# gregspangenberg/shoulder

Measured on AMD Instinct MI355X. Metric: humerus meshes/s end-to-end (all 4 landmarks), higher is better.
Workload: dtype f64 geometry + bf16 UNet

## Files before the change

shoulder_amd/csrc/k_ovf.h:

```cpp
#pragma once
#include "k_slices.h"

namespace sh {

struct OvfPools {
  Seg* segs; double* ring; unsigned char* work;
  unsigned long long seg_cap, ring_cap, work_cap;
  unsigned long long* ctr;
  int open_mode;
};
__host__ __device__ inline int ovf_nodes(int cnt, int open_mode) { return open_mode ? 2 * cnt : cnt; }

struct OvfSet { long long* soff; long long* roff; long long* woff; int* fill; int* list; int* nlist ; int* list2; };

__host__ __device__ inline unsigned ovf_hash_size(int n) { unsigned h = 64; while (h < 2u * (unsigned)n) h <<= 1; return h; }
__host__ __device__ inline unsigned long long ovf_work_bytes(int n) {
  unsigned long long b = (unsigned long long)n * 8ull * 5ull + (unsigned long long)ovf_hash_size(n) * 4ull + (unsigned long long)n * 4ull * 6ull + 64ull;
  const unsigned long long te = (unsigned long long)(n + 1) * 8ull * 7ull + 64ull;
  if (te > b) b = te;
  return (b + 15ull) & ~15ull;
}

__global__ void k_ovf_plan(int N, int nplanes, const int* __restrict__ seg_count, OvfPools P, OvfSet S, int* __restrict__ err) {
  const int pl = blockIdx.x * blockDim.x + threadIdx.x;
// ... 277 lines not shown
      const int qq = q == L ? 0 : q;
      const int src = rev ? (qq == 0 ? 0 : L - qq) : qq;
      ring_out[2 * q] = rx[o + src];
      ring_out[2 * q + 1] = ry[o + src];
    }
  }
  __syncthreads();
}

template <bool OPEN>
__global__ void __launch_bounds__(SH_HUGE_THREADS)
k_slice_link_huge(int N, const int* __restrict__ seg_count, OvfPools P, OvfSet S, double* __restrict__ centroids, double* __restrict__ areas,
                  int* __restrict__ nloops, int* __restrict__ ring_n, int want_ring, int select, int* __restrict__ err, double* __restrict__ areas_total,
                  const double* __restrict__ vobb, const long long* __restrict__ voff, const double* __restrict__ zeff, const OpenCfg oc) {
  const int nl = *S.nlist;
  for (int i = blockIdx.x; i < nl; i += gridDim.x) {
    const int pl = S.list[i];
    slice_link_plane_g<OPEN>(pl, N, seg_count, P.segs + S.soff[pl], vobb + 3 * voff[pl / N], zeff[pl], P.work + S.woff[pl], centroids, areas, nloops, ring_n,
                       want_ring ? P.ring + 2 * S.roff[pl] : (double*)nullptr, select, err, areas_total, oc);
  }
}

__global__ void __launch_bounds__(SH_RS_THREADS)
k_resample_polar_huge(int N, int M, const int* __restrict__ ring_n, OvfPools P, OvfSet S, const double* __restrict__ centroids,
                      double* __restrict__ ixy, double* __restrict__ itr_start, double* __restrict__ itr_cs, const RsWant W) {
  constexpr int NS = SH_MPROX / SH_RS_THREADS;
  __shared__ int amin_idx;
  __shared__ double wmin[SH_RS_THREADS / 64];
  __shared__ int widx[SH_RS_THREADS / 64];
  const int nlist = *S.nlist, tid = threadIdx.x;
  for (int it = blockIdx.x; it < nlist; it += gridDim.x) {
    const int pl = S.list[it];
    const int kpl = pl % N;
    const bool want_st = W.keep_all || kpl >= W.st_lo, want_cs = W.keep_all || (kpl >= W.cs_lo && kpl < W.cs_hi);
    if (!want_st && !want_cs) continue;
    const int L = ring_n[pl];
    const double* rp = P.ring + 2 * S.roff[pl];
    double* d = (double*)(P.work + S.woff[pl]);
    for (int q = 1 + tid; q <= L; q += SH_RS_THREADS) {
      const double dx = rp[2 * q] - rp[2 * (q - 1)], dy = rp[2 * q + 1] - rp[2 * (q - 1) + 1];
      d[q] = sqrt(dx * dx + dy * dy);
    }
    __syncthreads();
    if (tid == 0) {
      double acc = 0.0;
      d[0] = 0.0;
      for (int q = 1; q <= L; ++q) { acc += d[q]; d[q] = acc; }
    }
    __syncthreads();
    const double dmax = d[L];
    double sx[NS], sy[NS];
#pragma unroll
    for (int u = 0; u < NS; ++u) {
      const int j = tid + u * SH_RS_THREADS;
      const double t = linspace_at(0.0, dmax, M, j);
      const int n = L + 1;
      if (t < d[0]) { sx[u] = rp[0]; sy[u] = rp[1]; }
      else if (!(t < d[n - 1])) { sx[u] = rp[2 * (n - 1)]; sy[u] = rp[2 * (n - 1) + 1]; }
      else {
        int lo = 0, hi = n - 1;
        while (hi - lo > 1) { const int mid = (lo + hi) >> 1; if (t >= d[mid]) lo = mid; else hi = mid; }
        const double x0 = d[lo], fx = rp[2 * lo], fy = rp[2 * lo + 1];
        if (x0 == t) { sx[u] = fx; sy[u] = fy; }
        else {
          const double den = d[lo + 1] - x0;
          sx[u] = (rp[2 * (lo + 1)] - fx) / den * (t - x0) + fx;
          sy[u] = (rp[2 * (lo + 1) + 1] - fy) / den * (t - x0) + fy;
        }
      }
    }
    if (W.keep_all) {
      double* oxy = ixy + (size_t)pl * 2 * M;
#pragma unroll
      for (int u = 0; u < NS; ++u) { const int j = tid + u * SH_RS_THREADS; oxy[j] = sx[u]; oxy[M + j] = sy[u]; }
    }
    const double cx = centroids[2 * (size_t)pl], cy = centroids[2 * (size_t)pl + 1];
    for (int pass = 0; pass < 2; ++pass) {
      if (pass == 0 ? !want_st : !want_cs) continue;
      const double ox = pass ? cx : 0.0, oy = pass ? cy : 0.0;
      double best = 1e300;
      int bi = 0x7fffffff;
      double th[NS], rr[NS];
#pragma unroll
      for (int u = 0; u < NS; ++u) {
        const int j = tid + u * SH_RS_THREADS;
        const double x = sx[u] - ox, y = sy[u] - oy;
        th[u] = atan2(y, x);
        rr[u] = sqrt(x * x + y * y);
        if (th[u] < best || (th[u] == best && j < bi)) { best = th[u]; bi = j; }
      }
      for (int off = 32; off > 0; off >>= 1) {
        const double ob = __shfl_down(best, off);
        const int oi = __shfl_down(bi, off);
        if (ob < best || (ob == best && oi < bi)) { best = ob; bi = oi; }
      }
      if ((tid & 63) == 0) { wmin[tid >> 6] = best; widx[tid >> 6] = bi; }
      __syncthreads();
      if (tid == 0) {
        double bv = wmin[0]; int bx = widx[0];
        for (int w = 1; w < SH_RS_THREADS / 64; ++w)
          if (wmin[w] < bv || (wmin[w] == bv && widx[w] < bx)) { bv = wmin[w]; bx = widx[w]; }
        amin_idx = bx;
      }
      __syncthreads();
      const int k0 = amin_idx;
      double* o = (pass ? itr_cs : itr_start) + (size_t)pl * 2 * M;
#pragma unroll
      for (int u = 0; u < NS; ++u) {
        int dst = tid + u * SH_RS_THREADS - k0; if (dst < 0) dst += M;
        o[dst] = th[u];
        o[M + dst] = rr[u];
      }
      __syncthreads();
    }
  }
}

}
```

shoulder_amd/csrc/k_slices.h:

```cpp
#pragma once
#include "sh_demand.h"
#include "sh_scalar.h"
#include "sh_cutmath.h"

namespace sh {

struct __attribute__((aligned(16))) Seg {
  uint32_t s_lo, s_hi, e_lo, e_hi;
};
static_assert(sizeof(Seg) == 16, "Seg must be 16 bytes");
__device__ inline void seg_start_point(const double* __restrict__ vb , uint32_t lo, uint32_t hi, double z, double* x, double* y) {
  const double* pl = vb + 3 * (size_t)lo;
  const double* ph = vb + 3 * (size_t)hi;
  const double dl = pl[2] - z, dh = ph[2] - z;
  const double t = dl / (dl - dh);
  *x = pl[0] + t * (ph[0] - pl[0]);
  *y = pl[1] + t * (ph[1] - pl[1]);
}

__device__ inline unsigned long long enc_f64(double v) {
  unsigned long long b = (unsigned long long)__double_as_longlong(v);
  return (b & 0x8000000000000000ull) ? ~b : (b | 0x8000000000000000ull);
}
__device__ inline double dec_f64(unsigned long long e) {
// ... 99 lines not shown
    return;
  }
  if (kind == 0) { a = 0.99 * zmax; e = 0.99 * zmin; }
  else if (kind == 1) { a = 0.99 * zmax; e = neck_z[b]; }
  else { a = 0.99 * zmin; e = 0.0; }
  double* z = zs + (size_t)b * N;
  for (int k = threadIdx.x; k < N; k += blockDim.x) z[k] = linspace_at(a, e, N, k);
  __syncthreads();
  __shared__ double z_orig;
  if (threadIdx.x == 0) z_orig = np_pairwise_sum(z, N) / (double)N;
  __syncthreads();
  for (int k = threadIdx.x; k < N; k += blockDim.x) zeff[(size_t)b * N + k] = z_orig + (z[k] - z_orig);
}

#define SH_EMIT_MAXN 640
__global__ void __launch_bounds__(256)
k_slice_emit(const double* __restrict__ vobb, const int* __restrict__ faces,
             const long long* __restrict__ voff, const long long* __restrict__ foff, SliceSets sets) {
  __shared__ int hist[SH_EMIT_MAXN];
  int b = blockIdx.y;
  long long f0 = foff[b], nf = foff[b + 1] - f0;
  const double* vb = vobb + 3 * voff[b];
  const int nsets = sets.n, Ntot = sets.s[0].N + (nsets > 1 ? sets.s[1].N : 0);
  for (long long f_base = blockIdx.x * (long long)blockDim.x; f_base < nf; f_base += (long long)gridDim.x * blockDim.x) {
    for (int k = threadIdx.x; k < Ntot; k += blockDim.x) hist[k] = 0;
    const long long fi = f_base + threadIdx.x;
    const bool live = fi < nf;
    const int* f = faces + 3 * (f0 + (live ? fi : 0));
    int id[3] = {f[0], f[1], f[2]};
    double Z[3];
    for (int k = 0; k < 3; ++k) Z[k] = vb[3 * (size_t)id[k] + 2];
    double fzmin = fmin(Z[0], fmin(Z[1], Z[2])), fzmax = fmax(Z[0], fmax(Z[1], Z[2]));
    int lo_[2] = {1, 1}, hi_[2] = {0, 0};
    for (int si = 0; si < nsets; ++si) {
      const int N = sets.s[si].N;
      const double* zp = sets.s[si].zeff + (size_t)b * N;
      const double z_first = zp[0], z_last = zp[N - 1];
      const double inv_step = (double)(N - 1) / (z_last - z_first);
      double ka = (fzmin - z_first) * inv_step, kb = (fzmax - z_first) * inv_step;
      double klo = fmin(ka, kb), khi = fmax(ka, kb);
      int lo = 1, hi = 0;
      if (live && !(khi < -1.0 || klo > (double)N)) {
        lo = (int)floor(fmax(klo, 0.0)) - 1; hi = (int)ceil(fmin(khi, (double)(N - 1))) + 1;
        lo = lo < 0 ? 0 : lo;
        hi = hi > N - 1 ? N - 1 : hi;
      }
      if (live && N == 1) { lo = 0; hi = 0; }
      lo_[si] = lo; hi_[si] = hi;
    }
    __syncthreads();
    for (int si = 0; si < nsets; ++si) {
      const int N = sets.s[si].N, hoff = si ? sets.s[0].N : 0;
      const double* zp = sets.s[si].zeff + (size_t)b * N;
      for (int k = lo_[si]; k <= hi_[si]; ++k) {
        const double z = zp[k];
        const int s0 = Z[0] - z < -SH_SECTION_TOL ? -1 : 1, s1 = Z[1] - z < -SH_SECTION_TOL ? -1 : 1, s2 = Z[2] - z < -SH_SECTION_TOL ? -1 : 1;
        if (!(s0 == s1 && s1 == s2)) atomicAdd(&hist[hoff + k], 1);
      }
    }
    __syncthreads();
    for (int k = threadIdx.x; k < Ntot; k += blockDim.x) {
      const int n = hist[k];
      if (n > 0) {
        const int si = k >= sets.s[0].N ? 1 : 0, kk = si ? k - sets.s[0].N : k;
        hist[k] = atomicAdd(&sets.s[si].seg_count[(size_t)b * sets.s[si].N + kk], n);
      }
    }
    __syncthreads();
    for (int si = 0; si < nsets; ++si) {
      const int N = sets.s[si].N, hoff = si ? sets.s[0].N : 0;
      const double* zp = sets.s[si].zeff + (size_t)b * N;
      Seg* segs = sets.s[si].segs;
      for (int k = lo_[si]; k <= hi_[si]; ++k) {
        const double z = zp[k];
        double d[3];
        int s[3];
        for (int j = 0; j < 3; ++j) { d[j] = Z[j] - z; s[j] = d[j] < -SH_SECTION_TOL ? -1 : 1; }
        if (s[0] == s[1] && s[1] == s[2]) continue;
        const int slot = atomicAdd(&hist[hoff + k], 1);
        int up = 0, dn = 0;
        for (int j = 0; j < 3; ++j) {
          int jn = (j + 1) % 3;
          if (s[j] == -1 && s[jn] == 1) up = j;
          if (s[j] == 1 && s[jn] == -1) dn = j;
        }
        Seg sg;
        {
          int a = dn, c = (dn + 1) % 3;
          int l = id[a] < id[c] ? a : c, h = id[a] < id[c] ? c : a;
          sg.s_lo = (uint32_t)id[l]; sg.s_hi = (uint32_t)id[h];
        }
        {
          int a = up, c = (up + 1) % 3;
          int l = id[a] < id[c] ? a : c, h = id[a] < id[c] ? c : a;
          sg.e_lo = (uint32_t)id[l]; sg.e_hi = (uint32_t)id[h];
        }
        if (slot < SH_MAXSEG) segs[((size_t)b * N + k) * SH_MAXSEG + slot] = sg;
      }
    }
    __syncthreads();
  }
}

#define SH_LINK_THREADS 256
#define SH_SMALLSEG 384

template <int T>
__device__ inline int bridge_open_chains(const int n, const int cap, const int maxe, unsigned long long* __restrict__ skey,
                                         const unsigned long long* __restrict__ ekey, int* __restrict__ nxt, int* __restrict__ pred,
                                         int* __restrict__ ctl, int* tl, int* hd, int* bt, int* bh, int* mt, int* mh,
                                         double* tx, double* ty, double* hx, double* hy,
                                         const double* __restrict__ vb, const double z, const double max_gap) {
  const int tid = threadIdx.x;
  for (int i = tid; i < n; i += T) pred[i] = 0;
  if (tid < 4) ctl[tid] = 0;
  __syncthreads();
  for (int i = tid; i < n; i += T) if (nxt[i] != i) atomicAdd(&pred[nxt[i]], 1);
  __syncthreads();
  for (int i = tid; i < n; i += T) {
    if (nxt[i] == i) { const int q = atomicAdd(&ctl[0], 1); if (q < maxe) tl[q] = i; }
    if (pred[i] == 0) { const int q = atomicAdd(&ctl[1], 1); if (q < maxe) hd[q] = i; }
  }
  __syncthreads();
  const int nt = ctl[0], nh = ctl[1];
  if (nt > maxe || nh > maxe) return -1;
// ... 27 lines not shown
          if (best < 0 || d < bd || (d == bd && k < bk)) { best = t; bd = d; bk = k; }
        }
      bh[q] = best;
    }
    __syncthreads();
    for (int q = tid; q < nt; q += T) {
      const int h = bt[q];
      if (h >= 0 && bh[h] == q) { mt[q] = h; mh[h] = q; ctl[2] = 1; }
    }
    __syncthreads();
    if (ctl[2] == 0) break;
  }
  for (int q = tid; q < nt; q += T)
    if (mt[q] >= 0) {
      const int v = n + atomicAdd(&ctl[3], 1);
      if (v < cap) { skey[v] = ekey[tl[q]]; nxt[v] = hd[mt[q]]; nxt[tl[q]] = v; }
    }
  __syncthreads();
  const int nb = ctl[3];
  return n + nb > cap ? -1 : n + nb;
}


template <int CAP, bool OPEN>
__device__ inline void slice_link_plane(const int pl, int N, const int* __restrict__ seg_count, const Seg* __restrict__ segs,
             const double* __restrict__ vobb, const long long* __restrict__ voff, const double* __restrict__ zeff,
             double* __restrict__ centroids, double* __restrict__ areas, int* __restrict__ nloops,
             int* __restrict__ ring_n, double* __restrict__ ring , int select, int* __restrict__ err,
             double* __restrict__ areas_total , ManyLoops many, const OpenCfg oc,
             int* __restrict__ nlarge = nullptr) {
  constexpr int HASH = CAP <= 384 ? 512 : 2048;
  static_assert(HASH * 4 <= CAP * 8 && HASH > CAP, "the hash table lives in bufB");
  __shared__ unsigned long long skey[CAP];
  __shared__ unsigned long long bufA[CAP];
  __shared__ unsigned long long bufB[CAP];
  __shared__ int nxt[CAP], jmpA[CAP], jmpB[CAP], offA[CAP], offB[CAP];
  int* const table = (int*)bufB;
  __shared__ unsigned long long l_key[SH_MAXLOOPS];
  __shared__ int l_start[SH_MAXLOOPS], l_len[SH_MAXLOOPS], l_off[SH_MAXLOOPS];
  __shared__ double l_area[SH_MAXLOOPS], l_sel[SH_MAXLOOPS];
  __shared__ int n_loops, bad;
  __shared__ double bbv[4];

  const int b = pl / N;
  const int tid = threadIdx.x;
  int cnt = seg_count[pl];
  if (CAP == SH_SMALLSEG ? cnt > SH_SMALLSEG : cnt <= SH_SMALLSEG) {
    if (CAP == SH_SMALLSEG && nlarge && tid == 0) atomicAdd(nlarge, 1);
    return;
  }
  if (cnt > SH_MAXSEG) return;
  const int n = cnt;
  if (tid == 0) { n_loops = 0; bad = 0; }
  for (int i = tid; i < HASH; i += SH_LINK_THREADS) table[i] = -1;
  const Seg* sp = segs + (size_t)pl * SH_MAXSEG;
  const double* vb = vobb + 3 * voff[b];
  const double zpl = zeff[pl];
  for (int i = tid; i < n; i += SH_LINK_THREADS) {
    Seg s = sp[i];
    skey[i] = ((unsigned long long)s.s_lo << 32) | s.s_hi;
    bufA[i] = ((unsigned long long)s.e_lo << 32) | s.e_hi;
  }
  __syncthreads();
  if (n < 3 && !(OPEN && n > 0)) {
    if (tid == 0) {
      centroids[2 * (size_t)pl] = 0; centroids[2 * (size_t)pl + 1] = 0; areas[pl] = 0; nloops[pl] = 0; ring_n[pl] = 0;
      if (areas_total) areas_total[pl] = 0;
      else atomicCAS(&err[b], 0, SH_ERR_GEOMETRY_DEV);
    }
    return;
  }
  for (int i = tid; i < n; i += SH_LINK_THREADS) {
    uint32_t h = hash_key64(skey[i]) & (HASH - 1);
    while (atomicCAS(&table[h], -1, i) != -1) h = (h + 1) & (HASH - 1);
  }
// ... 153 lines not shown
  }
  __syncthreads();
  int best = 0;
  for (int l = 1; l < nl; ++l) {
    if (select == 0) { if (fabs(l_area[l]) > fabs(l_area[best])) best = l; }
    else { if (l_sel[l] < l_sel[best]) best = l; }
  }
  if (tid == 0) {
    double x0 = bbv[0], x1 = bbv[1], y0 = bbv[2], y1 = bbv[3];
    centroids[2 * (size_t)pl] = 0.5 * (x0 + x1);
    centroids[2 * (size_t)pl + 1] = 0.5 * (y0 + y1);
    int amax = 0;
    for (int l = 1; l < nl; ++l) if (fabs(l_area[l]) > fabs(l_area[amax])) amax = l;
    areas[pl] = fabs(l_area[amax]);
    if (areas_total) {
      double tot = 0.0;
      for (int l = 0; l < nl; ++l) tot += l_area[l];
      areas_total[pl] = fabs(tot);
    }
    nloops[pl] = nl;
    ring_n[pl] = l_len[best];
    if (bad) atomicCAS(&err[b], 0, SH_ERR_GEOMETRY_DEV);
  }
  if (ring) {
    int l = best, o = l_off[l], L = l_len[l];
    bool rev = l_area[l] < 0;
    double* out = ring + (size_t)pl * (SH_MAXSEG + 1) * 2;
    for (int q = tid; q <= L; q += SH_LINK_THREADS) {
      int qq = q == L ? 0 : q;
      int src = rev ? (qq == 0 ? 0 : L - qq) : qq;
      out[2 * q] = rx[o + src];
      out[2 * q + 1] = ry[o + src];
    }
  }
}

template <bool OPEN>
__global__ void __launch_bounds__(SH_LINK_THREADS)
k_slice_link(SliceSets sets, int B, int* __restrict__ err) {
  const int ntot = sets.s[0].N + (sets.n > 1 ? sets.s[1].N : 0);
  int id = (int)blockIdx.x;
  if (B % 8 == 0) { const int x = id & 7, j = id >> 3; id = (x + 8 * (j / ntot)) * ntot + j % ntot; }
  const int b = id / ntot, kk = id - b * ntot;
  const int si = kk >= sets.s[0].N ? 1 : 0;
  const SliceSetDev& S = sets.s[si];
  slice_link_plane<SH_SMALLSEG, OPEN>(b * S.N + (kk - (si ? sets.s[0].N : 0)), S.N, S.seg_count, S.segs, sets.vobb, sets.voff, S.zeff, S.centroids, S.areas, S.nloops, S.ring_n,
                                S.ring, S.select, err, S.areas_total, S.many, sets.open, S.nlarge);
}
template <bool OPEN>
__global__ void __launch_bounds__(SH_LINK_THREADS)
k_slice_link_large(SliceSets sets, int B, int* __restrict__ err) {
  for (int si = 0; si < sets.n; ++si) {
    const SliceSetDev& S = sets.s[si];
    if (*S.nlarge == 0) continue;
    const int nplanes = B * S.N;
    for (int pl = blockIdx.x; pl < nplanes; pl += gridDim.x) {
      const int cnt = S.seg_count[pl];
      if (cnt > SH_MAXSEG && S.ovf_missed && threadIdx.x == 0) atomicExch(S.ovf_missed, 1ull);
      if (cnt <= SH_SMALLSEG || cnt > SH_MAXSEG) continue;
      slice_link_plane<SH_MAXSEG, OPEN>(pl, S.N, S.seg_count, S.segs, sets.vobb, sets.voff, S.zeff, S.centroids, S.areas, S.nloops, S.ring_n, S.ring, S.select, err, S.areas_total, S.many, sets.open);
      __syncthreads();
    }
  }
}

#define SH_RS_THREADS 128
struct RsWant { int keep_all, st_lo, cs_lo, cs_hi; };
template <int CAP>
__device__ inline void resample_polar_plane(const int pl, int N, int M, const int* __restrict__ ring_n, const double* __restrict__ ring,
                 const double* __restrict__ centroids, double* __restrict__ ixy,
                 double* __restrict__ itr_start, double* __restrict__ itr_cs, const long long* __restrict__ ovf_roff, const RsWant W) {
  static_assert(SH_MPROX % SH_RS_THREADS == 0, "whole samples per lane");
  constexpr int NS = SH_MPROX / SH_RS_THREADS;
  __shared__ double rx[CAP + 1], ry[CAP + 1], d[CAP + 1];
  __shared__ int amin_idx;
  __shared__ double wmin[SH_RS_THREADS / 64];
  __shared__ int widx[SH_RS_THREADS / 64];
  const int tid = threadIdx.x;
  const int L = ring_n[pl];
  if (CAP == SH_SMALLSEG ? L > SH_SMALLSEG : L <= SH_SMALLSEG) return;
  if (ovf_roff[pl] >= 0) return;
  const int kpl = pl % N;
  const bool want_st = W.keep_all || kpl >= W.st_lo, want_cs = W.keep_all || (kpl >= W.cs_lo && kpl < W.cs_hi);
  if (!want_st && !want_cs) return;
  const double* rp = ring + (size_t)pl * (SH_MAXSEG + 1) * 2;
  for (int q = tid; q <= L; q += SH_RS_THREADS) { rx[q] = rp[2 * q]; ry[q] = rp[2 * q + 1]; }
  __syncthreads();
  for (int q = 1 + tid; q <= L; q += SH_RS_THREADS) {
    double dx = rx[q] - rx[q - 1], dy = ry[q] - ry[q - 1];
    d[q] = sqrt(dx * dx + dy * dy);
  }
  __syncthreads();
  if (tid == 0) {
    double acc = 0.0;
    d[0] = 0.0;
    int q = 1;
    for (; q + 8 <= L + 1; q += 8) {
      double v[8];
#pragma unroll
      for (int u = 0; u < 8; ++u) v[u] = d[q + u];
#pragma unroll
      for (int u = 0; u < 8; ++u) { acc += v[u]; v[u] = acc; }
#pragma unroll
      for (int u = 0; u < 8; ++u) d[q + u] = v[u];
    }
    for (; q <= L; ++q) { acc += d[q]; d[q] = acc; }
  }
  __syncthreads();
  const double dmax = d[L];
  double sx[NS], sy[NS];
#pragma unroll
  for (int u = 0; u < NS; ++u) {
    const int j = tid + u * SH_RS_THREADS;
    const double t = linspace_at(0.0, dmax, M, j);
    const int n = L + 1;
    if (t < d[0]) { sx[u] = rx[0]; sy[u] = ry[0]; }
    else if (!(t < d[n - 1])) { sx[u] = rx[n - 1]; sy[u] = ry[n - 1]; }
    else {
      int lo = 0, hi = n - 1;
      while (hi - lo > 1) { const int mid = (lo + hi) >> 1; if (t >= d[mid]) lo = mid; else hi = mid; }
      const double x0 = d[lo], fx = rx[lo], fy = ry[lo];
      if (x0 == t) { sx[u] = fx; sy[u] = fy; }
      else {
        const double den = d[lo + 1] - x0;
        sx[u] = (rx[lo + 1] - fx) / den * (t - x0) + fx;
        sy[u] = (ry[lo + 1] - fy) / den * (t - x0) + fy;
      }
    }
  }
  if (W.keep_all) {
    double* oxy = ixy + (size_t)pl * 2 * M;
#pragma unroll
    for (int u = 0; u < NS; ++u) { const int j = tid + u * SH_RS_THREADS; oxy[j] = sx[u]; oxy[M + j] = sy[u]; }
  }
  const double cx = centroids[2 * (size_t)pl], cy = centroids[2 * (size_t)pl + 1];
  for (int pass = 0; pass < 2; ++pass) {
    if (pass == 0 ? !want_st : !want_cs) continue;
    const double ox = pass ? cx : 0.0, oy = pass ? cy : 0.0;
    double best = 1e300;
    int bi = 0x7fffffff;
    double th[NS], rr[NS];
#pragma unroll
    for (int u = 0; u < NS; ++u) {
      const int j = tid + u * SH_RS_THREADS;
      const double x = sx[u] - ox, y = sy[u] - oy;
      th[u] = atan2(y, x);
      rr[u] = sqrt(x * x + y * y);
      if (th[u] < best || (th[u] == best && j < bi)) { best = th[u]; bi = j; }
    }
    for (int off = 32; off > 0; off >>= 1) {
      double ob = __shfl_down(best, off);
      int oi = __shfl_down(bi, off);
      if (ob < best || (ob == best && oi < bi)) { best = ob; bi = oi; }
    }
    if ((tid & 63) == 0) { wmin[tid >> 6] = best; widx[tid >> 6] = bi; }
    __syncthreads();
    if (tid == 0) {
      double bv = wmin[0]; int bx = widx[0];
      for (int w = 1; w < SH_RS_THREADS / 64; ++w)
        if (wmin[w] < bv || (wmin[w] == bv && widx[w] < bx)) { bv = wmin[w]; bx = widx[w]; }
      amin_idx = bx;
    }
    __syncthreads();
    const int k0 = amin_idx;
    double* o = (pass ? itr_cs : itr_start) + (size_t)pl * 2 * M;
#pragma unroll
    for (int u = 0; u < NS; ++u) {
      int dst = tid + u * SH_RS_THREADS - k0; if (dst < 0) dst += M;
      o[dst] = th[u];
      o[M + dst] = rr[u];
    }
    __syncthreads();
  }
}

__global__ void __launch_bounds__(SH_RS_THREADS)
k_resample_polar(int N, int M, const int* __restrict__ ring_n, const double* __restrict__ ring, const double* __restrict__ centroids,
                 double* __restrict__ ixy, double* __restrict__ itr_start, double* __restrict__ itr_cs, const long long* __restrict__ ovf_roff, const RsWant W) {
  resample_polar_plane<SH_SMALLSEG>(blockIdx.x, N, M, ring_n, ring, centroids, ixy, itr_start, itr_cs, ovf_roff, W);
}
__global__ void __launch_bounds__(SH_RS_THREADS)
k_resample_polar_large(int nplanes, int N, int M, const int* __restrict__ ring_n, const double* __restrict__ ring, const double* __restrict__ centroids,
                       double* __restrict__ ixy, double* __restrict__ itr_start, double* __restrict__ itr_cs, const int* __restrict__ nlarge,
                       const long long* __restrict__ ovf_roff, const RsWant W) {
  if (*nlarge == 0) return;
  for (int pl = blockIdx.x; pl < nplanes; pl += gridDim.x) {
    if (ring_n[pl] <= SH_SMALLSEG || ovf_roff[pl] >= 0) continue;
    resample_polar_plane<SH_MAXSEG>(pl, N, M, ring_n, ring, centroids, ixy, itr_start, itr_cs, ovf_roff, W);
    __syncthreads();
  }
}

}
```

shoulder_amd/csrc/shoulder_hip.hip:

```cpp
#include "sh_ctx.h"

#include "k_slices.h"
#include "k_ovf.h"
#include "k_open.h"
#include "k_stages.h"
#include "k_groove.h"
#include "k_anp.h"
#include "k_stl.h"
#include "k_clip.h"
#include "k_resect.h"
#include "k_headfit.h"
#include "k_seat.h"
#include "k_stem.h"
#include "k_plan.h"
#include "k_te.h"
#include "k_obb.h"
#include "sh_hull.h"

#include <sched.h>

using namespace sh;

struct FillList { void* p[6]; unsigned long long n[6]; unsigned v[6]; };
__global__ void k_fill_list(FillList L) {
// ... 1177 lines not shown
    const SliceSetView& a = v.set[sp.id];
    { int orc; if ((orc = ovf_set(c, def.pfx, def.N, &OS[i])) != SH_OK) return orc; }
    SliceSetDev& S = sets.s[i];
    S.N = def.N; S.kind = sp.kind; S.select = sp.select;
    S.zb = sp.kind == 4 ? v.obb_zb_pre : v.z_bounds;
    S.zs = a.zs; S.zeff = a.zeff; S.seg_count = a.seg_count; S.segs = a.segs;
    S.centroids = a.centroids; S.areas = a.areas; S.nloops = a.nloops; S.ring_n = a.ring_n;
    S.ring = a.ring; S.areas_total = a.area_total;
    S.nlarge = v.slices_nlarge + (sp.kind & 7);
    S.many = ManyLoops{ovf_on ? OS[i].list2 : (int*)nullptr, ovf_on ? OS[i].nlist + 1 : (int*)nullptr, ovf_on ? (unsigned long long*)nullptr : OP.ctr + SH_CTR_TIER_MISSED};
    S.ovf_missed = ovf_on ? (unsigned long long*)nullptr : OP.ctr + SH_CTR_TIER_MISSED;
    S.aux = PlaneAux{sp.decode_bounds ? (const unsigned long long*)v.zb_enc : (const unsigned long long*)nullptr, v.z_bounds, S.seg_count, S.nlarge,
                     ovf_on ? OS[i].nlist : (int*)nullptr, i == 0 ? OP.ctr : (unsigned long long*)nullptr};
  }
  LAUNCH(c, "k_make_planes", k_make_planes, dim3(B, nspec), dim3(256), sets, (const double*)v.neck_z, B);
  dim3 g((unsigned)std::min<long long>((c->maxF + 255) / 256, 4096), (unsigned)B);
  LAUNCH(c, "k_slice_emit", k_slice_emit, g, dim3(256), v.verts_obb, v.faces, v.voff, v.foff, sets);
  if (ovf_on)
    for (int i = 0; i < nspec; ++i) {
      const SliceSetDev& S = sets.s[i];
      LAUNCH(c, "k_ovf_plan", k_ovf_plan, dim3((unsigned)((B * S.N + 255) / 256)), dim3(256), S.N, B * S.N, (const int*)S.seg_count, OP, OS[i], v.err);
      LAUNCH(c, "k_slice_emit_ovf", k_slice_emit_ovf, g, dim3(256), v.verts_obb, v.faces, v.voff, v.foff, (const double*)S.zeff, S.N, OP, OS[i]);
    }
  LAUNCH(c, "k_slice_link", bridge ? k_slice_link<true> : k_slice_link<false>, dim3(B * ntot), dim3(SH_LINK_THREADS), sets, B, v.err);
  LAUNCH(c, "k_slice_link_large", bridge ? k_slice_link_large<true> : k_slice_link_large<false>, dim3(std::min(B * ntot, 512)), dim3(SH_LINK_THREADS), sets, B, v.err);
  for (int i = 0; i < nspec; ++i) {
    const SliceSpec& sp = specs[i];
    const SliceSetDev& S = sets.s[i];
    if (ovf_on) {
      LAUNCH(c, "k_ovf_plan_loops", k_ovf_plan_loops, dim3(16), dim3(256), S.N, (const int*)S.seg_count, (const Seg*)S.segs, OP, OS[i], v.err);
      LAUNCH(c, "k_slice_link_huge", bridge ? k_slice_link_huge<true> : k_slice_link_huge<false>, dim3(64), dim3(SH_HUGE_THREADS), S.N, (const int*)S.seg_count, OP, OS[i],
             S.centroids, S.areas, S.nloops, S.ring_n, SLICE_SETS[sp.id].ring ? 1 : 0, S.select, v.err, S.areas_total, (const double*)v.verts_obb, (const long long*)v.voff,
             (const double*)S.zeff, sets.open);
    }
    if (sp.resample) {
      RsWant want{c->keep_products ? 1 : 0, SH_ANP_ROW0, 0, 0};
      cutoff_range(SH_NPROX, c->params.groove_cutoff[0], c->params.groove_cutoff[1], &want.cs_lo, &want.cs_hi);
      if (c->b0 == 0) { c->rs_cs_lo = want.cs_lo; c->rs_cs_hi = want.cs_hi; c->rs_all = c->keep_products; c->rs_gen = c->batch_gen; }
#define RS_ROWS S.centroids, v.prox_ixy, v.prox_itr_start, v.prox_itr_centered_start
      LAUNCH(c, "k_resample_polar", k_resample_polar, dim3(B * S.N), dim3(SH_RS_THREADS), S.N, SH_MPROX, S.ring_n, S.ring, RS_ROWS, (const long long*)OS[i].roff, want);
      LAUNCH(c, "k_resample_polar_large", k_resample_polar_large, dim3(std::min(B * S.N, 512)), dim3(SH_RS_THREADS), B * S.N, S.N, SH_MPROX, S.ring_n, S.ring, RS_ROWS,
             (const int*)S.nlarge, (const long long*)OS[i].roff, want);
      if (ovf_on) LAUNCH(c, "k_resample_polar_huge", k_resample_polar_huge, dim3(64), dim3(SH_RS_THREADS), S.N, SH_MPROX, (const int*)S.ring_n, OP, OS[i], RS_ROWS, want);
#undef RS_ROWS
    }
  }
  return SH_OK;
}
static int run_slice_set(sh_ctx* c, const WinView& v, const SliceSpec& sp) { return run_slice_sets(c, v, &sp, 1); }
static SliceSpec spec_full(bool decode) { return {SET_FULL, 0, false, 0, decode}; }
static SliceSpec spec_distal(bool decode) { return {SET_DISTAL, 2, false, 0, decode}; }
static const SliceSpec SPEC_PROX = {SET_PROX, 1, true, 0, false}, SPEC_NECKC = {SET_NECKC, 3, false, 1, false}, SPEC_POBB = {SET_POBB, 4, false, 0, false};

static bool hull_fits(const sh_ctx* c, int slot, int B, int* need ) {
  const int* counts = c->hstage[slot].cnt;
  int nvmax = 1, nfmax = 1, nemax = 1;
  for (int b = 0; b < B; ++b) { nvmax = std::max(nvmax, counts[b]); nfmax = std::max(nfmax, counts[B + b]); nemax = std::max(nemax, counts[2 * B + b]); }
  if (need) { need[0] = nvmax; need[1] = nfmax; need[2] = nemax; }
  return nvmax <= c->hcap.v && nfmax <= c->hcap.f && nemax <= c->hcap.e;
}
static int grow_hull_records(sh_ctx* c, int nv, int nf, int ne) {
  auto up = [](int x) { return (x + x / 8 + 1023) / 1024 * 1024; };
  HIPCHK(c, hipStreamSynchronize(c->stream));
  if (nv > c->hcap.v) c->hcap.v = up(nv);
  if (nf > c->hcap.f) c->hcap.f = up(nf);
  if (ne > c->hcap.e) c->hcap.e = up(ne);
  int rc;
// ... 1084 lines not shown
```

Baseline: 9165.

## Fuse polar resampling into small-tier slice linking and window emit histogram

Polar resampling of small-tier planes now runs inside the slice-link kernel. The ring is kept in LDS arrays unioned with the join's dead scratch, which removes a separate k_resample_polar launch and a global ring round-trip. The emit kernel also tracks a per-block active plane window, so it only scans and clears that histogram range and skips iterations where no face hits a plane. The costs are more code, higher LDS pressure in the link kernel, and resampling now runs on 256-thread blocks instead of 128.

After: 8800. 0.96x the previous value.

```diff
diff --git a/shoulder_amd/csrc/k_ovf.h b/shoulder_amd/csrc/k_ovf.h
--- a/shoulder_amd/csrc/k_ovf.h
+++ b/shoulder_amd/csrc/k_ovf.h
@@ -323,98 +323,16 @@
 }
 
 __global__ void __launch_bounds__(SH_RS_THREADS)
-k_resample_polar_huge(int N, int M, const int* __restrict__ ring_n, OvfPools P, OvfSet S, const double* __restrict__ centroids,
-                      double* __restrict__ ixy, double* __restrict__ itr_start, double* __restrict__ itr_cs, const RsWant W) {
-  constexpr int NS = SH_MPROX / SH_RS_THREADS;
-  __shared__ int amin_idx;
-  __shared__ double wmin[SH_RS_THREADS / 64];
-  __shared__ int widx[SH_RS_THREADS / 64];
-  const int nlist = *S.nlist, tid = threadIdx.x;
+k_resample_polar_huge(int N, int M, const int* __restrict__ ring_n, OvfPools P, OvfSet S, const double* __restrict__ centroids, const RsRows O, const RsWant W) {
+  const int nlist = *S.nlist;
   for (int it = blockIdx.x; it < nlist; it += gridDim.x) {
     const int pl = S.list[it];
     const int kpl = pl % N;
     const bool want_st = W.keep_all || kpl >= W.st_lo, want_cs = W.keep_all || (kpl >= W.cs_lo && kpl < W.cs_hi);
     if (!want_st && !want_cs) continue;
-    const int L = ring_n[pl];
-    const double* rp = P.ring + 2 * S.roff[pl];
-    double* d = (double*)(P.work + S.woff[pl]);
-    for (int q = 1 + tid; q <= L; q += SH_RS_THREADS) {
-      const double dx = rp[2 * q] - rp[2 * (q - 1)], dy = rp[2 * q + 1] - rp[2 * (q - 1) + 1];
-      d[q] = sqrt(dx * dx + dy * dy);
-    }
-    __syncthreads();
-    if (tid == 0) {
-      double acc = 0.0;
-      d[0] = 0.0;
-      for (int q = 1; q <= L; ++q) { acc += d[q]; d[q] = acc; }
-    }
-    __syncthreads();
-    const double dmax = d[L];
-    double sx[NS], sy[NS];
-#pragma unroll
-    for (int u = 0; u < NS; ++u) {
-      const int j = tid + u * SH_RS_THREADS;
-      const double t = linspace_at(0.0, dmax, M, j);
-      const int n = L + 1;
-      if (t < d[0]) { sx[u] = rp[0]; sy[u] = rp[1]; }
-      else if (!(t < d[n - 1])) { sx[u] = rp[2 * (n - 1)]; sy[u] = rp[2 * (n - 1) + 1]; }
-      else {
-        int lo = 0, hi = n - 1;
-        while (hi - lo > 1) { const int mid = (lo + hi) >> 1; if (t >= d[mid]) lo = mid; else hi = mid; }
-        const double x0 = d[lo], fx = rp[2 * lo], fy = rp[2 * lo + 1];
-        if (x0 == t) { sx[u] = fx; sy[u] = fy; }
-        else {
-          const double den = d[lo + 1] - x0;
-          sx[u] = (rp[2 * (lo + 1)] - fx) / den * (t - x0) + fx;
-          sy[u] = (rp[2 * (lo + 1) + 1] - fy) / den * (t - x0) + fy;
-        }
-      }
-    }
-    if (W.keep_all) {
-      double* oxy = ixy + (size_t)pl * 2 * M;
-#pragma unroll
-      for (int u = 0; u < NS; ++u) { const int j = tid + u * SH_RS_THREADS; oxy[j] = sx[u]; oxy[M + j] = sy[u]; }
-    }
-    const double cx = centroids[2 * (size_t)pl], cy = centroids[2 * (size_t)pl + 1];
-    for (int pass = 0; pass < 2; ++pass) {
-      if (pass == 0 ? !want_st : !want_cs) continue;
-      const double ox = pass ? cx : 0.0, oy = pass ? cy : 0.0;
-      double best = 1e300;
-      int bi = 0x7fffffff;
-      double th[NS], rr[NS];
-#pragma unroll
-      for (int u = 0; u < NS; ++u) {
-        const int j = tid + u * SH_RS_THREADS;
-        const double x = sx[u] - ox, y = sy[u] - oy;
-        th[u] = atan2(y, x);
-        rr[u] = sqrt(x * x + y * y);
-        if (th[u] < best || (th[u] == best && j < bi)) { best = th[u]; bi = j; }
-      }
-      for (int off = 32; off > 0; off >>= 1) {
-        const double ob = __shfl_down(best, off);
-        const int oi = __shfl_down(bi, off);
-        if (ob < best || (ob == best && oi < bi)) { best = ob; bi = oi; }
-      }
-      if ((tid & 63) == 0) { wmin[tid >> 6] = best; widx[tid >> 6] = bi; }
-      __syncthreads();
-      if (tid == 0) {
-        double bv = wmin[0]; int bx = widx[0];
-        for (int w = 1; w < SH_RS_THREADS / 64; ++w)
-          if (wmin[w] < bv || (wmin[w] == bv && widx[w] < bx)) { bv = wmin[w]; bx = widx[w]; }
-        amin_idx = bx;
-      }
-      __syncthreads();
-      const int k0 = amin_idx;
-      double* o = (pass ? itr_cs : itr_start) + (size_t)pl * 2 * M;
-#pragma unroll
-      for (int u = 0; u < NS; ++u) {
-        int dst = tid + u * SH_RS_THREADS - k0; if (dst < 0) dst += M;
-        o[dst] = th[u];
-        o[M + dst] = rr[u];
-      }
-      __syncthreads();
-    }
-  }
-}
-
-}
+    resample_polar_rows<SH_RS_THREADS>(RingPairs{P.ring + 2 * S.roff[pl]}, (double*)(P.work + S.woff[pl]), ring_n[pl], M, centroids[2 * (size_t)pl],
+                                       centroids[2 * (size_t)pl + 1], (size_t)pl, O, W.keep_all != 0, want_st, want_cs);
+  }
+}
+
+}
diff --git a/shoulder_amd/csrc/k_slices.h b/shoulder_amd/csrc/k_slices.h
--- a/shoulder_amd/csrc/k_slices.h
+++ b/shoulder_amd/csrc/k_slices.h
@@ -145,8 +145,13 @@
   long long f0 = foff[b], nf = foff[b + 1] - f0;
   const double* vb = vobb + 3 * voff[b];
   const int nsets = sets.n, Ntot = sets.s[0].N + (nsets > 1 ? sets.s[1].N : 0);
-  for (long long f_base = blockIdx.x * (long long)blockDim.x; f_base < nf; f_base += (long long)gridDim.x * blockDim.x) {
-    for (int k = threadIdx.x; k < Ntot; k += blockDim.x) hist[k] = 0;
+  __shared__ int win[2][2];
+  for (int k = threadIdx.x; k < Ntot; k += blockDim.x) hist[k] = 0;
+  if (threadIdx.x == 0) { win[0][0] = SH_EMIT_MAXN; win[0][1] = -1; }
+  __syncthreads();
+  int par = 0;
+  for (long long f_base = blockIdx.x * (long long)blockDim.x; f_base < nf; f_base += (long long)gridDim.x * blockDim.x, par ^= 1) {
+    if (threadIdx.x == 0) { win[par ^ 1][0] = SH_EMIT_MAXN; win[par ^ 1][1] = -1; }
     const long long fi = f_base + threadIdx.x;
     const bool live = fi < nf;
     const int* f = faces + 3 * (f0 + (live ? fi : 0));
@@ -171,7 +176,14 @@
       if (live && N == 1) { lo = 0; hi = 0; }
       lo_[si] = lo; hi_[si] = hi;
     }
-    __syncthreads();
+    int w0 = SH_EMIT_MAXN, w1 = -1;
+    for (int si = 0; si < nsets; ++si)
+      if (lo_[si] <= hi_[si]) { const int hoff = si ? sets.s[0].N : 0; w0 = min(w0, hoff + lo_[si]); w1 = max(w1, hoff + hi_[si]); }
+    const bool mine = w1 >= 0;
+    for (int off = 32; off > 0; off >>= 1) { w0 = min(w0, __shfl_xor(w0, off)); w1 = max(w1, __shfl_xor(w1, off)); }
+    if ((threadIdx.x & 63) == 0 && w1 >= 0) { atomicMin(&win[par][0], w0); atomicMax(&win[par][1], w1); }
+    if (!__syncthreads_or(mine)) continue;
+    w0 = win[par][0]; w1 = win[par][1];
     for (int si = 0; si < nsets; ++si) {
       const int N = sets.s[si].N, hoff = si ? sets.s[0].N : 0;
       const double* zp = sets.s[si].zeff + (size_t)b * N;
@@ -182,7 +194,7 @@
       }
     }
     __syncthreads();
-    for (int k = threadIdx.x; k < Ntot; k += blockDim.x) {
+    for (int k = w0 + threadIdx.x; k <= w1; k += blockDim.x) {
       const int n = hist[k];
       if (n > 0) {
         const int si = k >= sets.s[0].N ? 1 : 0, kk = si ? k - sets.s[0].N : k;
@@ -222,8 +234,115 @@
       }
     }
     __syncthreads();
-  }
-}
+    for (int k = w0 + threadIdx.x; k <= w1; k += blockDim.x) hist[k] = 0;
+  }
+}
+
+#define SH_RS_THREADS 128
+struct RsWant { int keep_all, st_lo, cs_lo, cs_hi; };
+struct RsRows { double* ixy; double* itr_start; double* itr_cs; };
+struct RingXY { const double* rx; const double* ry;
+  __device__ double x(int q) const { return rx[q]; }
+  __device__ double y(int q) const { return ry[q]; } };
+struct RingPairs { const double* rp;
+  __device__ double x(int q) const { return rp[2 * q]; }
+  __device__ double y(int q) const { return rp[2 * q + 1]; } };
+template <int T, class Ring>
+__device__ inline void resample_polar_rows(const Ring R, double* d, const int L, const int M, const double cx, const double cy,
+                                           const size_t pl, const RsRows O, const bool keep_all, const bool want_st, const bool want_cs) {
+  static_assert(SH_MPROX % T == 0 && T % 64 == 0, "whole samples per lane, whole waves");
+  constexpr int NS = SH_MPROX / T;
+  __shared__ int amin_idx;
+  __shared__ double wmin[T / 64];
+  __shared__ int widx[T / 64];
+  const int tid = threadIdx.x;
+  for (int q = 1 + tid; q <= L; q += T) {
+    double dx = R.x(q) - R.x(q - 1), dy = R.y(q) - R.y(q - 1);
+    d[q] = sqrt(dx * dx + dy * dy);
+  }
+  __syncthreads();
+  if (tid == 0) {
+    double acc = 0.0;
+    d[0] = 0.0;
+    int q = 1;
+    for (; q + 8 <= L + 1; q += 8) {
+      double v[8];
+#pragma unroll
+      for (int u = 0; u < 8; ++u) v[u] = d[q + u];
+#pragma unroll
+      for (int u = 0; u < 8; ++u) { acc += v[u]; v[u] = acc; }
+#pragma unroll
+      for (int u = 0; u < 8; ++u) d[q + u] = v[u];
+    }
+    for (; q <= L; ++q) { acc += d[q]; d[q] = acc; }
+  }
+  __syncthreads();
+  const double dmax = d[L];
+  double sx[NS], sy[NS];
+#pragma unroll
+  for (int u = 0; u < NS; ++u) {
+    const int j = tid + u * T;
+    const double t = linspace_at(0.0, dmax, M, j);
+    const int n = L + 1;
+    if (t < d[0]) { sx[u] = R.x(0); sy[u] = R.y(0); }
+    else if (!(t < d[n - 1])) { sx[u] = R.x(n - 1); sy[u] = R.y(n - 1); }
+    else {
+      int lo = 0, hi = n - 1;
+      while (hi - lo > 1) { const int mid = (lo + hi) >> 1; if (t >= d[mid]) lo = mid; else hi = mid; }
+      const double x0 = d[lo], fx = R.x(lo), fy = R.y(lo);
+      if (x0 == t) { sx[u] = fx; sy[u] = fy; }
+      else {
+        const double den = d[lo + 1] - x0;
+        sx[u] = (R.x(lo + 1) - fx) / den * (t - x0) + fx;
+        sy[u] = (R.y(lo + 1) - fy) / den * (t - x0) + fy;
+      }
+    }
+  }
+  if (keep_all) {
+    double* oxy = O.ixy + pl * 2 * M;
+#pragma unroll
+    for (int u = 0; u < NS; ++u) { const int j = tid + u * T; oxy[j] = sx[u]; oxy[M + j] = sy[u]; }
+  }
+  for (int pass = 0; pass < 2; ++pass) {
+    if (pass == 0 ? !want_st : !want_cs) continue;
+    const double ox = pass ? cx : 0.0, oy = pass ? cy : 0.0;
+    double best = 1e300;
+    int bi = 0x7fffffff;
+    double th[NS], rr[NS];
+#pragma unroll
+    for (int u = 0; u < NS; ++u) {
+      const int j = tid + u * T;
+      const double x = sx[u] - ox, y = sy[u] - oy;
+      th[u] = atan2(y, x);
+      rr[u] = sqrt(x * x + y * y);
+      if (th[u] < best || (th[u] == best && j < bi)) { best = th[u]; bi = j; }
+    }
+    for (int off = 32; off > 0; off >>= 1) {
+      double ob = __shfl_down(best, off);
+      int oi = __shfl_down(bi, off);
+      if (ob < best || (ob == best && oi < bi)) { best = ob; bi = oi; }
+    }
+    if ((tid & 63) == 0) { wmin[tid >> 6] = best; widx[tid >> 6] = bi; }
+    __syncthreads();
+    if (tid == 0) {
+      double bv = wmin[0]; int bx = widx[0];
+      for (int w = 1; w < T / 64; ++w)
+        if (wmin[w] < bv || (wmin[w] == bv && widx[w] < bx)) { bv = wmin[w]; bx = widx[w]; }
+      amin_idx = bx;
+    }
+    __syncthreads();
+    const int k0 = amin_idx;
+    double* o = (pass ? O.itr_cs : O.itr_start) + pl * 2 * M;
+#pragma unroll
+    for (int u = 0; u < NS; ++u) {
+      int dst = tid + u * T - k0; if (dst < 0) dst += M;
+      o[dst] = th[u];
+      o[M + dst] = rr[u];
+    }
+    __syncthreads();
+  }
+}
+struct RsFuse { int M; RsWant W; RsRows O; const long long* ovf_roff; };
 
 #define SH_LINK_THREADS 256
 #define SH_SMALLSEG 384
@@ -297,19 +416,31 @@
 }
 
 
-template <int CAP, bool OPEN>
+template <int CAP>
+struct LinkLds {
+  unsigned long long bufA[CAP];
+  unsigned long long bufB[CAP];
+  union {
+    struct { unsigned long long skey[CAP]; int nxt[CAP], jmpA[CAP], jmpB[CAP], offA[CAP], offB[CAP]; } j;
+    struct { double x[CAP + 1], y[CAP + 1], d[CAP + 1]; } r;
+  };
+};
+template <int CAP, bool OPEN, bool FUSE = false>
 __device__ inline void slice_link_plane(const int pl, int N, const int* __restrict__ seg_count, const Seg* __restrict__ segs,
              const double* __restrict__ vobb, const long long* __restrict__ voff, const double* __restrict__ zeff,
              double* __restrict__ centroids, double* __restrict__ areas, int* __restrict__ nloops,
              int* __restrict__ ring_n, double* __restrict__ ring , int select, int* __restrict__ err,
              double* __restrict__ areas_total , ManyLoops many, const OpenCfg oc,
-             int* __restrict__ nlarge = nullptr) {
+             int* __restrict__ nlarge = nullptr, const RsFuse rf = RsFuse{}) {
+  static_assert(!FUSE || CAP == SH_SMALLSEG, "the large tier's planes are resampled by k_resample_polar_large");
+  static_assert(sizeof(((LinkLds<CAP>*)nullptr)->r) <= sizeof(((LinkLds<CAP>*)nullptr)->j), "the ring fits in the join's dead arrays");
   constexpr int HASH = CAP <= 384 ? 512 : 2048;
   static_assert(HASH * 4 <= CAP * 8 && HASH > CAP, "the hash table lives in bufB");
-  __shared__ unsigned long long skey[CAP];
-  __shared__ unsigned long long bufA[CAP];
-  __shared__ unsigned long long bufB[CAP];
-  __shared__ int nxt[CAP], jmpA[CAP], jmpB[CAP], offA[CAP], offB[CAP];
+  __shared__ LinkLds<CAP> lds;
+  unsigned long long* const skey = lds.j.skey;
+  unsigned long long* const bufA = lds.bufA;
+  unsigned long long* const bufB = lds.bufB;
+  int* const nxt = lds.j.nxt; int* const jmpA = lds.j.jmpA; int* const jmpB = lds.j.jmpB; int* const offA = lds.j.offA; int* const offB = lds.j.offB;
   int* const table = (int*)bufB;
   __shared__ unsigned long long l_key[SH_MAXLOOPS];
   __shared__ int l_start[SH_MAXLOOPS], l_len[SH_MAXLOOPS], l_off[SH_MAXLOOPS];
@@ -326,6 +457,7 @@
   }
   if (cnt > SH_MAXSEG) return;
   const int n = cnt;
+  const bool rs_here = FUSE && rf.ovf_roff[pl] < 0;
   if (tid == 0) { n_loops = 0; bad = 0; }
   for (int i = tid; i < HASH; i += SH_LINK_THREADS) table[i] = -1;
   const Seg* sp = segs + (size_t)pl * SH_MAXSEG;
@@ -525,30 +657,42 @@
     ring_n[pl] = l_len[best];
     if (bad) atomicCAS(&err[b], 0, SH_ERR_GEOMETRY_DEV);
   }
-  if (ring) {
+  bool rows = false, want_st = false, want_cs = false;
+  if (rs_here && l_len[best] <= CAP) {
+    const int kpl = pl - b * N;
+    want_st = rf.W.keep_all || kpl >= rf.W.st_lo; want_cs = rf.W.keep_all || (kpl >= rf.W.cs_lo && kpl < rf.W.cs_hi);
+    rows = want_st || want_cs;
+  }
+  if (ring || rows) {
     int l = best, o = l_off[l], L = l_len[l];
     bool rev = l_area[l] < 0;
-    double* out = ring + (size_t)pl * (SH_MAXSEG + 1) * 2;
+    double* out = ring ? ring + (size_t)pl * (SH_MAXSEG + 1) * 2 : nullptr;
     for (int q = tid; q <= L; q += SH_LINK_THREADS) {
       int qq = q == L ? 0 : q;
       int src = rev ? (qq == 0 ? 0 : L - qq) : qq;
-      out[2 * q] = rx[o + src];
-      out[2 * q + 1] = ry[o + src];
-    }
-  }
-}
-
-template <bool OPEN>
+      const double vx = rx[o + src], vy = ry[o + src];
+      if (out) { out[2 * q] = vx; out[2 * q + 1] = vy; }
+      if (FUSE && rows) { lds.r.x[q] = vx; lds.r.y[q] = vy; }
+    }
+  }
+  if (FUSE && rows) {
+    __syncthreads();
+    resample_polar_rows<SH_LINK_THREADS>(RingXY{lds.r.x, lds.r.y}, lds.r.d, l_len[best], rf.M, 0.5 * (bbv[0] + bbv[1]), 0.5 * (bbv[2] + bbv[3]),
+                                         (size_t)pl, rf.O, rf.W.keep_all != 0, want_st, want_cs);
+  }
+}
+
+template <bool OPEN, bool FUSE>
 __global__ void __launch_bounds__(SH_LINK_THREADS)
-k_slice_link(SliceSets sets, int B, int* __restrict__ err) {
+k_slice_link(SliceSets sets, int B, int* __restrict__ err, RsFuse rf) {
   const int ntot = sets.s[0].N + (sets.n > 1 ? sets.s[1].N : 0);
   int id = (int)blockIdx.x;
   if (B % 8 == 0) { const int x = id & 7, j = id >> 3; id = (x + 8 * (j / ntot)) * ntot + j % ntot; }
   const int b = id / ntot, kk = id - b * ntot;
   const int si = kk >= sets.s[0].N ? 1 : 0;
   const SliceSetDev& S = sets.s[si];
-  slice_link_plane<SH_SMALLSEG, OPEN>(b * S.N + (kk - (si ? sets.s[0].N : 0)), S.N, S.seg_count, S.segs, sets.vobb, sets.voff, S.zeff, S.centroids, S.areas, S.nloops, S.ring_n,
-                                S.ring, S.select, err, S.areas_total, S.many, sets.open, S.nlarge);
+  slice_link_plane<SH_SMALLSEG, OPEN, FUSE>(b * S.N + (kk - (si ? sets.s[0].N : 0)), S.N, S.seg_count, S.segs, sets.vobb, sets.voff, S.zeff, S.centroids, S.areas, S.nloops, S.ring_n,
+                                      S.ring, S.select, err, S.areas_total, S.many, sets.open, S.nlarge, rf);
 }
 template <bool OPEN>
 __global__ void __launch_bounds__(SH_LINK_THREADS)
@@ -567,131 +711,28 @@
   }
 }
 
-#define SH_RS_THREADS 128
-struct RsWant { int keep_all, st_lo, cs_lo, cs_hi; };
 template <int CAP>
 __device__ inline void resample_polar_plane(const int pl, int N, int M, const int* __restrict__ ring_n, const double* __restrict__ ring,
-                 const double* __restrict__ centroids, double* __restrict__ ixy,
-                 double* __restrict__ itr_start, double* __restrict__ itr_cs, const long long* __restrict__ ovf_roff, const RsWant W) {
-  static_assert(SH_MPROX % SH_RS_THREADS == 0, "whole samples per lane");
-  constexpr int NS = SH_MPROX / SH_RS_THREADS;
+                 const double* __restrict__ centroids, const RsRows O, const RsWant W) {
   __shared__ double rx[CAP + 1], ry[CAP + 1], d[CAP + 1];
-  __shared__ int amin_idx;
-  __shared__ double wmin[SH_RS_THREADS / 64];
-  __shared__ int widx[SH_RS_THREADS / 64];
   const int tid = threadIdx.x;
   const int L = ring_n[pl];
-  if (CAP == SH_SMALLSEG ? L > SH_SMALLSEG : L <= SH_SMALLSEG) return;
-  if (ovf_roff[pl] >= 0) return;
   const int kpl = pl % N;
   const bool want_st = W.keep_all || kpl >= W.st_lo, want_cs = W.keep_all || (kpl >= W.cs_lo && kpl < W.cs_hi);
   if (!want_st && !want_cs) return;
   const double* rp = ring + (size_t)pl * (SH_MAXSEG + 1) * 2;
   for (int q = tid; q <= L; q += SH_RS_THREADS) { rx[q] = rp[2 * q]; ry[q] = rp[2 * q + 1]; }
   __syncthreads();
-  for (int q = 1 + tid; q <= L; q += SH_RS_THREADS) {
-    double dx = rx[q] - rx[q - 1], dy = ry[q] - ry[q - 1];
-    d[q] = sqrt(dx * dx + dy * dy);
-  }
-  __syncthreads();
-  if (tid == 0) {
-    double acc = 0.0;
-    d[0] = 0.0;
-    int q = 1;
-    for (; q + 8 <= L + 1; q += 8) {
-      double v[8];
-#pragma unroll
-      for (int u = 0; u < 8; ++u) v[u] = d[q + u];
-#pragma unroll
-      for (int u = 0; u < 8; ++u) { acc += v[u]; v[u] = acc; }
-#pragma unroll
-      for (int u = 0; u < 8; ++u) d[q + u] = v[u];
-    }
-    for (; q <= L; ++q) { acc += d[q]; d[q] = acc; }
-  }
-  __syncthreads();
-  const double dmax = d[L];
-  double sx[NS], sy[NS];
-#pragma unroll
-  for (int u = 0; u < NS; ++u) {
-    const int j = tid + u * SH_RS_THREADS;
-    const double t = linspace_at(0.0, dmax, M, j);
-    const int n = L + 1;
-    if (t < d[0]) { sx[u] = rx[0]; sy[u] = ry[0]; }
-    else if (!(t < d[n - 1])) { sx[u] = rx[n - 1]; sy[u] = ry[n - 1]; }
-    else {
-      int lo = 0, hi = n - 1;
-      while (hi - lo > 1) { const int mid = (lo + hi) >> 1; if (t >= d[mid]) lo = mid; else hi = mid; }
-      const double x0 = d[lo], fx = rx[lo], fy = ry[lo];
-      if (x0 == t) { sx[u] = fx; sy[u] = fy; }
-      else {
-        const double den = d[lo + 1] - x0;
-        sx[u] = (rx[lo + 1] - fx) / den * (t - x0) + fx;
-        sy[u] = (ry[lo + 1] - fy) / den * (t - x0) + fy;
-      }
-    }
-  }
-  if (W.keep_all) {
-    double* oxy = ixy + (size_t)pl * 2 * M;
-#pragma unroll
-    for (int u = 0; u < NS; ++u) { const int j = tid + u * SH_RS_THREADS; oxy[j] = sx[u]; oxy[M + j] = sy[u]; }
-  }
-  const double cx = centroids[2 * (size_t)pl], cy = centroids[2 * (size_t)pl + 1];
-  for (int pass = 0; pass < 2; ++pass) {
-    if (pass == 0 ? !want_st : !want_cs) continue;
-    const double ox = pass ? cx : 0.0, oy = pass ? cy : 0.0;
-    double best = 1e300;
-    int bi = 0x7fffffff;
-    double th[NS], rr[NS];
-#pragma unroll
-    for (int u = 0; u < NS; ++u) {
-      const int j = tid + u * SH_RS_THREADS;
-      const double x = sx[u] - ox, y = sy[u] - oy;
-      th[u] = atan2(y, x);
-      rr[u] = sqrt(x * x + y * y);
-      if (th[u] < best || (th[u] == best && j < bi)) { best = th[u]; bi = j; }
-    }
-    for (int off = 32; off > 0; off >>= 1) {
-      double ob = __shfl_down(best, off);
-      int oi = __shfl_down(bi, off);
-      if (ob < best || (ob == best && oi < bi)) { best = ob; bi = oi; }
-    }
-    if ((tid & 63) == 0) { wmin[tid >> 6] = best; widx[tid >> 6] = bi; }
-    __syncthreads();
-    if (tid == 0) {
-      double bv = wmin[0]; int bx = widx[0];
-      for (int w = 1; w < SH_RS_THREADS / 64; ++w)
-        if (wmin[w] < bv || (wmin[w] == bv && widx[w] < bx)) { bv = wmin[w]; bx = widx[w]; }
-      amin_idx = bx;
-    }
-    __syncthreads();
-    const int k0 = amin_idx;
-    double* o = (pass ? itr_cs : itr_start) + (size_t)pl * 2 * M;
-#pragma unroll
-    for (int u = 0; u < NS; ++u) {
-      int dst = tid + u * SH_RS_THREADS - k0; if (dst < 0) dst += M;
-      o[dst] = th[u];
-      o[M + dst] = rr[u];
-    }
-    __syncthreads();
-  }
-}
-
+  resample_polar_rows<SH_RS_THREADS>(RingXY{rx, ry}, d, L, M, centroids[2 * (size_t)pl], centroids[2 * (size_t)pl + 1], (size_t)pl, O, W.keep_all != 0, want_st, want_cs);
+}
 __global__ void __launch_bounds__(SH_RS_THREADS)
-k_resample_polar(int N, int M, const int* __restrict__ ring_n, const double* __restrict__ ring, const double* __restrict__ centroids,
-                 double* __restrict__ ixy, double* __restrict__ itr_start, double* __restrict__ itr_cs, const long long* __restrict__ ovf_roff, const RsWant W) {
-  resample_polar_plane<SH_SMALLSEG>(blockIdx.x, N, M, ring_n, ring, centroids, ixy, itr_start, itr_cs, ovf_roff, W);
-}
-__global__ void __launch_bounds__(SH_RS_THREADS)
-k_resample_polar_large(int nplanes, int N, int M, const int* __restrict__ ring_n, const double* __restrict__ ring, const double* __restrict__ centroids,
-                       double* __restrict__ ixy, double* __restrict__ itr_start, double* __restrict__ itr_cs, const int* __restrict__ nlarge,
-                       const long long* __restrict__ ovf_roff, const RsWant W) {
+k_resample_polar_large(int nplanes, int N, int M, const int* __restrict__ seg_count, const int* __restrict__ ring_n, const double* __restrict__ ring,
+                       const double* __restrict__ centroids, const RsRows O, const int* __restrict__ nlarge, const long long* __restrict__ ovf_roff, const RsWant W) {
   if (*nlarge == 0) return;
   for (int pl = blockIdx.x; pl < nplanes; pl += gridDim.x) {
-    if (ring_n[pl] <= SH_SMALLSEG || ovf_roff[pl] >= 0) continue;
-    resample_polar_plane<SH_MAXSEG>(pl, N, M, ring_n, ring, centroids, ixy, itr_start, itr_cs, ovf_roff, W);
-    __syncthreads();
-  }
-}
-
-}
+    if ((seg_count[pl] <= SH_SMALLSEG && ring_n[pl] <= SH_SMALLSEG) || ovf_roff[pl] >= 0) continue;
+    resample_polar_plane<SH_MAXSEG>(pl, N, M, ring_n, ring, centroids, O, W);
+  }
+}
+
+}
diff --git a/shoulder_amd/csrc/shoulder_hip.hip b/shoulder_amd/csrc/shoulder_hip.hip
--- a/shoulder_amd/csrc/shoulder_hip.hip
+++ b/shoulder_amd/csrc/shoulder_hip.hip
@@ -1223,7 +1223,28 @@
       LAUNCH(c, "k_ovf_plan", k_ovf_plan, dim3((unsigned)((B * S.N + 255) / 256)), dim3(256), S.N, B * S.N, (const int*)S.seg_count, OP, OS[i], v.err);
       LAUNCH(c, "k_slice_emit_ovf", k_slice_emit_ovf, g, dim3(256), v.verts_obb, v.faces, v.voff, v.foff, (const double*)S.zeff, S.N, OP, OS[i]);
     }
-  LAUNCH(c, "k_slice_link", bridge ? k_slice_link<true> : k_slice_link<false>, dim3(B * ntot), dim3(SH_LINK_THREADS), sets, B, v.err);
+  int rs_set = -1;
+  RsWant want{c->keep_products ? 1 : 0, SH_ANP_ROW0, 0, 0};
+  const RsRows rows{v.prox_ixy, v.prox_itr_start, v.prox_itr_centered_start};
+  for (int i = 0; i < nspec; ++i)
+    if (specs[i].resample) {
+      cutoff_range(SH_NPROX, c->params.groove_cutoff[0], c->params.groove_cutoff[1], &want.cs_lo, &want.cs_hi);
+      if (c->b0 == 0) { c->rs_cs_lo = want.cs_lo; c->rs_cs_hi = want.cs_hi; c->rs_all = c->keep_products; c->rs_gen = c->batch_gen; }
+      rs_set = i;
+    }
+  if (rs_set < 0) {
+    LAUNCH(c, "k_slice_link", (bridge ? k_slice_link<true, false> : k_slice_link<false, false>), dim3(B * ntot), dim3(SH_LINK_THREADS), sets, B, v.err, RsFuse{});
+  } else {
+    SliceSets one = sets;
+    one.n = 1;
+    if (nspec == 2) {
+      one.s[0] = sets.s[1 - rs_set];
+      LAUNCH(c, "k_slice_link", (bridge ? k_slice_link<true, false> : k_slice_link<false, false>), dim3(B * one.s[0].N), dim3(SH_LINK_THREADS), one, B, v.err, RsFuse{});
+    }
+    one.s[0] = sets.s[rs_set];
+    const RsFuse rf{SH_MPROX, want, rows, (const long long*)OS[rs_set].roff};
+    LAUNCH(c, "k_resample_polar", (bridge ? k_slice_link<true, true> : k_slice_link<false, true>), dim3(B * one.s[0].N), dim3(SH_LINK_THREADS), one, B, v.err, rf);
+  }
   LAUNCH(c, "k_slice_link_large", bridge ? k_slice_link_large<true> : k_slice_link_large<false>, dim3(std::min(B * ntot, 512)), dim3(SH_LINK_THREADS), sets, B, v.err);
   for (int i = 0; i < nspec; ++i) {
     const SliceSpec& sp = specs[i];
@@ -1235,15 +1256,9 @@
              (const double*)S.zeff, sets.open);
     }
     if (sp.resample) {
-      RsWant want{c->keep_products ? 1 : 0, SH_ANP_ROW0, 0, 0};
-      cutoff_range(SH_NPROX, c->params.groove_cutoff[0], c->params.groove_cutoff[1], &want.cs_lo, &want.cs_hi);
-      if (c->b0 == 0) { c->rs_cs_lo = want.cs_lo; c->rs_cs_hi = want.cs_hi; c->rs_all = c->keep_products; c->rs_gen = c->batch_gen; }
-#define RS_ROWS S.centroids, v.prox_ixy, v.prox_itr_start, v.prox_itr_centered_start
-      LAUNCH(c, "k_resample_polar", k_resample_polar, dim3(B * S.N), dim3(SH_RS_THREADS), S.N, SH_MPROX, S.ring_n, S.ring, RS_ROWS, (const long long*)OS[i].roff, want);
-      LAUNCH(c, "k_resample_polar_large", k_resample_polar_large, dim3(std::min(B * S.N, 512)), dim3(SH_RS_THREADS), B * S.N, S.N, SH_MPROX, S.ring_n, S.ring, RS_ROWS,
-             (const int*)S.nlarge, (const long long*)OS[i].roff, want);
-      if (ovf_on) LAUNCH(c, "k_resample_polar_huge", k_resample_polar_huge, dim3(64), dim3(SH_RS_THREADS), S.N, SH_MPROX, (const int*)S.ring_n, OP, OS[i], RS_ROWS, want);
-#undef RS_ROWS
+      LAUNCH(c, "k_resample_polar_large", k_resample_polar_large, dim3(std::min(B * S.N, 512)), dim3(SH_RS_THREADS), B * S.N, S.N, SH_MPROX, (const int*)S.seg_count,
+             (const int*)S.ring_n, (const double*)S.ring, (const double*)S.centroids, rows, (const int*)S.nlarge, (const long long*)OS[i].roff, want);
+      if (ovf_on) LAUNCH(c, "k_resample_polar_huge", k_resample_polar_huge, dim3(64), dim3(SH_RS_THREADS), S.N, SH_MPROX, (const int*)S.ring_n, OP, OS[i], (const double*)S.centroids, rows, want);
     }
   }
   return SH_OK;
```
